# yoeripoels/neural-pde-surrogates

Hardware: AMD Instinct MI355X
Metric: rollout timesteps/sec on 256x256 two-phase grid (sample-timesteps/s); rel-L2 vs CPU reference (higher is better)
Workload: dtype f32 (1x1/2x2/3x3/5x5 convs: 3-pass split-fp16 MFMA); 1 GPU; UFNO twophase cfg rollout (simulate), 256x256, 3 fields, obstacle mask, tw=25; model=ufno, global_batch=16, per_gpu_batch=16, res=256, num_c=3, parallelism=dp1 (batch-sharded rollout, no collective)

## Files before the change

### neural-pde-surrogates_amd/csrc/conv2d_x3.hip

```cpp
#include "conv2d_common.hpp"

#include <cstdlib>
#include <type_traits>

namespace {

__host__ __device__ constexpr int x3_patch_px_max(int ntaps, int tile_px) {
    return ntaps == 1      ? tile_px
           : ntaps == 25   ? (tile_px == 512 ? 12 * 68 : 12 * 36)
           : tile_px == 128 ? (ntaps == 4 ? 5 * 33 : 6 * 34)
                            : (tile_px == 512 ? (ntaps == 4 ? 9 * 65 : 10 * 66) : (ntaps == 4 ? 9 * 33 : 10 * 34));
}

#define X3_MFMA __builtin_amdgcn_mfma_f32_32x32x16_f16
__device__ __forceinline__ int x3_slot_px(int idx) { return idx >> 2; }

template <int N, typename F>
__device__ __forceinline__ void static_for(F&& f) {
    if constexpr (N > 0) {
        static_for<N - 1>(f);
        f(std::integral_constant<int, N - 1>{});
    }
}

// ... 432 lines not shown
                        *reinterpret_cast<f32x4*>(T + P * (NCO + 4) + cw0 + cb * 32 + 8 * m + 4 * h) = v;
                    }
            }
            barrier();
            x3_store_phase<TILE_PX, NCO>(a, b, cob, oy0, ox0, g.T, ph, T, btab, tid, amax, reinterpret_cast<double*>(smem));
        } else if constexpr (!WIDE) {
            static_for<PBW>([&](auto pbc) {
                constexpr int pb = decltype(pbc)::value;
                const int P = px0 + pb * 32 + (lane & 31);
                const int ti = P / a.TW, tj = P - (P / a.TW) * a.TW;
                const int oy = oy0 + ti * g.T, ox = ox0 + tj * g.T;
                if (oy >= a.Hout || ox >= a.Wout) return;
                const int dy = oy * a.out_os + a.out_off_y + (ph >> 1), dx = ox * a.out_os + a.out_off_x + (ph & 1);
                if (dy < 0 || dy >= a.out_H || dx < 0 || dx >= a.out_W) return;
#pragma unroll
                for (int cb = 0; cb < CBW; ++cb) {
                    f32x16 v = acc[cb][pb];
#pragma unroll
                    for (int r = 0; r < 16; ++r) v[r] *= inv;
                    store_tile(a, b, cob * NCO + cw0 + cb * 32, h, v, dy, dx, amax);
                    __builtin_amdgcn_sched_barrier(0);
                }
            });
            barrier();
        }
        barrier();
    }
    nps::tag_publish(a.out_tag, amax, nps::wave_salt());
}



template <int PB, int D>
__global__ __launch_bounds__(512) void conv1x1_x3_kernel(const nps_conv2d_t a) {
    constexpr int CBW = 2;
    const int lane = threadIdx.x & 63, wv = threadIdx.x >> 6;
    const int co_lo = blockIdx.z * 512;
    const int cob = (co_lo >> 6) + wv;
    const int b = blockIdx.y;
    const int h = lane >> 5;
    const int npx = a.Hout * a.Wout;
    const int P0 = blockIdx.x * (PB * 32);
    const float xs = in_scale_of(a);
    const bool scaled = has_in_scale(a);
    int fy[PB], fx[PB];
    unsigned pin = 0;
#pragma unroll
    for (int pb = 0; pb < PB; ++pb) {
        const int P = P0 + pb * 32 + (lane & 31);
        const int oy = P / a.Wout, ox = P - (P / a.Wout) * a.Wout;
        const int ye = oy - a.pad_y, xe = ox - a.pad_x;
        const bool ok = P < npx && ye >= 0 && ye < a.Hin + 2 * a.circ && xe >= 0 && xe < a.Win + 2 * a.circ;
        fy[pb] = a.circ ? nps::wrap_mod(ye - a.circ, a.Hin) : ye;
        fx[pb] = a.circ ? nps::wrap_mod(xe - a.circ, a.Win) : xe;
        pin = ok ? (pin | (1u << pb)) : pin;
    }
    const float* sp[PB];
    int cur_src = -1;
    int cbase = 0;
    auto locate = [&](int sidx) {
        const nps_src_t S0 = a.src[0], S1 = a.src[1], S2 = a.src[2];
        const float* sptr = sidx == 0 ? S0.ptr : (sidx == 1 ? S1.ptr : S2.ptr);
        const int sC = sidx == 0 ? S0.C : (sidx == 1 ? S1.C : S2.C);
        const int sH = sidx == 0 ? S0.H : (sidx == 1 ? S1.H : S2.H);
        const int sW = sidx == 0 ? S0.W : (sidx == 1 ? S1.W : S2.W);
        const int soy = sidx == 0 ? S0.off_y : (sidx == 1 ? S1.off_y : S2.off_y);
        const int sox = sidx == 0 ? S0.off_x : (sidx == 1 ? S1.off_x : S2.off_x);
#pragma unroll
        for (int pb = 0; pb < PB; ++pb) {
            const int yy = fy[pb] - soy, xx = fx[pb] - sox;
            const bool ok = ((pin >> pb) & 1u) && yy >= 0 && yy < sH && xx >= 0 && xx < sW;
            sp[pb] = ok ? sptr + ((size_t)(b * sH + yy) * sW + xx) * sC : nullptr;
        }
    };
    const int nstages = (a.Cin + 2 * CK - 1) / (2 * CK);
    const int last = nstages - 1;
    f32x4 raw[D][PB][4];
    auto issue = [&](int st, bool live, f32x4 (&r)[PB][4]) {
        const int c0 = st * 2 * CK + h * CK;
        int sidx = 0, lo = 0, sb = 0;
#pragma unroll
        for (int si = 0; si < NPS_MAX_SRC; ++si) {
            if (si < a.nsrc) {
                const int hi = lo + a.src[si].C;
                if (c0 >= lo && c0 < hi) {
                    sidx = si;
                    sb = lo;
                }
                lo = hi;
            }
        }
        if (sidx != cur_src) {
            locate(sidx);
            cur_src = sidx;
            cbase = sb;
        }
#pragma unroll
        for (int q = 0; q < 4; ++q) {
            const bool chok = live && c0 + q * 4 < a.Cin;
#pragma unroll
            for (int pb = 0; pb < PB; ++pb) {
                const float* src = (chok && sp[pb] != nullptr) ? sp[pb] + (c0 - cbase + q * 4) : x3_zero16;
                r[pb][q] = *reinterpret_cast<const f32x4*>(src);
            }
        }
    };
    const int ncb = packed_ncb(a.Cout);
    const size_t gstride = (size_t)ncb * 2048;
    const int wcob = cob < ncb / CBW ? cob : ncb / CBW - 1;
    const char* wbase = reinterpret_cast<const char*>(a.wpack) + (size_t)wcob * CBW * 2048 + lane * 16;
    f16x8 Aw[2][2][CBW][2];
    auto loadA = [&](int st, f16x8 (&d)[2][CBW][2]) {
#pragma unroll
        for (int k = 0; k < 2; ++k) {
            const char* p = wbase + (size_t)(2 * st + k) * gstride;
#pragma unroll
            for (int cb = 0; cb < CBW; ++cb) {
                d[k][cb][0] = *reinterpret_cast<const f16x8*>(p + cb * 2048);
                d[k][cb][1] = *reinterpret_cast<const f16x8*>(p + cb * 2048 + 1024);
            }
        }
    };
    f32x16 acc[CBW][PB];
#pragma unroll
    for (int i = 0; i < CBW; ++i)
#pragma unroll
        for (int j = 0; j < PB; ++j)
#pragma unroll
            for (int r = 0; r < 16; ++r) acc[i][j][r] = 0.f;
    static_for<D - 1>([&](auto jc) {
        constexpr int j = decltype(jc)::value;
        issue(min(j, last), j <= last, raw[j]);
    });
    loadA(0, Aw[0]);
    const int npad = (nstages + D - 1) / D * D;
    for (int s0 = 0; s0 < npad; s0 += D) {
        static_for<D>([&](auto jc) {
            constexpr int j = decltype(jc)::value;
            constexpr int jn = (j + D - 1) % D;
            const int st = s0 + j;
            issue(min(st + D - 1, last), st + D - 1 <= last, raw[jn]);
            loadA(min(st + 1, last), Aw[(j + 1) & 1]);
            __builtin_amdgcn_sched_barrier(0);
            constexpr int r = j & 1;
#pragma unroll
            for (int k = 0; k < 2; ++k) {
                f16x8 Bh[PB], Bl[PB];
#pragma unroll
                for (int pb = 0; pb < PB; ++pb) {
                    f16x4 h0, l0, h1, l1;
                    f32x4 v0 = raw[j][pb][2 * k], v1 = raw[j][pb][2 * k + 1];
                    if (scaled) {
                        v0 *= xs;
                        v1 *= xs;
                    }
                    split4(v0, h0, l0);
                    split4(v1, h1, l1);
                    Bh[pb] = f16x8{h0[0], h0[1], h0[2], h0[3], h1[0], h1[1], h1[2], h1[3]};
                    Bl[pb] = f16x8{l0[0], l0[1], l0[2], l0[3], l1[0], l1[1], l1[2], l1[3]};
                }
#pragma unroll
                for (int cb = 0; cb < CBW; ++cb)
#pragma unroll
                    for (int pb = 0; pb < PB; ++pb)
                        acc[cb][pb] = X3_MFMA(Aw[r][k][cb][0], Bh[pb], acc[cb][pb], 0, 0, 0);
#pragma unroll
                for (int cb = 0; cb < CBW; ++cb)
#pragma unroll
                    for (int pb = 0; pb < PB; ++pb)
                        acc[cb][pb] = X3_MFMA(Aw[r][k][cb][0], Bl[pb], acc[cb][pb], 0, 0, 0);
#pragma unroll
                for (int cb = 0; cb < CBW; ++cb)
#pragma unroll
                    for (int pb = 0; pb < PB; ++pb)
                        acc[cb][pb] = X3_MFMA(Aw[r][k][cb][1], Bh[pb], acc[cb][pb], 0, 0, 0);
            }
        });
    }
    const float inv = 1.f / (pow2_scale_for(a.wpack[packed_body(a.Cout, a.Cin, 1)]) * xs);
    if (x3_lds_epilogue(a)) {
        extern __shared__ __attribute__((aligned(16))) float T[];
        const int pitch = (int)(blockDim.x) + 4;
#pragma unroll
        for (int pb = 0; pb < PB; ++pb) {
            const int P = pb * 32 + (lane & 31);
#pragma unroll
            for (int cb = 0; cb < CBW; ++cb)
#pragma unroll
                for (int m = 0; m < 4; ++m) {
                    const f32x4 v = {acc[cb][pb][4 * m] * inv, acc[cb][pb][4 * m + 1] * inv,
                                     acc[cb][pb][4 * m + 2] * inv, acc[cb][pb][4 * m + 3] * inv};
                    *reinterpret_cast<f32x4*>(T + P * pitch + wv * 64 + cb * 32 + 8 * m + 4 * h) = v;
                }
        }
        __syncthreads();
        const int nco = min(a.Cout - co_lo, (int)blockDim.x);
        const int C4 = nco >> 2;
        const bool fixq = ((int)blockDim.x % C4) == 0;
        const int pstep = fixq ? (int)blockDim.x / C4 : 0;
        int fp = fixq ? (int)threadIdx.x / C4 : 0;
        const int fcl = fixq ? ((int)threadIdx.x - fp * C4) * 4 : 0;
        int foy = (P0 + fp) / a.Wout, fox = (P0 + fp) - ((P0 + fp) / a.Wout) * a.Wout;
        float amax = 0.f;
        for (int i = threadIdx.x; i < PB * 32 * C4; i += blockDim.x) {
            int p, cl, oy, ox;
            if (fixq) {
                p = fp;
                cl = fcl;
                oy = foy;
                ox = fox;
                fp += pstep;
                fox += pstep;
                while (fox >= a.Wout) {
                    fox -= a.Wout;
                    ++foy;
                }
            } else {
                p = i / C4;
                cl = (i - (i / C4) * C4) * 4;
                oy = (P0 + p) / a.Wout;
                ox = (P0 + p) - ((P0 + p) / a.Wout) * a.Wout;
            }
            const int co0 = co_lo + cl;
            const int P = P0 + p;
            if (P >= npx) continue;
            const int dy = oy * a.out_os + a.out_off_y, dx = ox * a.out_os + a.out_off_x;
            if (dy < 0 || dy >= a.out_H || dx < 0 || dx >= a.out_W) continue;
            const f32x4 accv = *reinterpret_cast<const f32x4*>(T + p * pitch + cl);
            const size_t o = (((size_t)b * a.out_H + dy) * a.out_W + dx) * a.out_C + co0;
            const f32x4 z = {0.f, 0.f, 0.f, 0.f};
            const f32x4 bi = a.bias ? *reinterpret_cast<const f32x4*>(a.bias + co0) : z;
            const f32x4 a0 = a.addend0 ? *reinterpret_cast<const f32x4*>(a.addend0 + o) : z;
            const f32x4 a1 = a.addend1 ? *reinterpret_cast<const f32x4*>(a.addend1 + o) : z;
            const f32x4 ov = a.accumulate ? *reinterpret_cast<const f32x4*>(a.out + o) : z;
            f32x4 r;
#pragma unroll
            for (int e = 0; e < 4; ++e) {
                float v = accv[e] + bi[e];
                if (!a.add_after_act) v = v + a0[e] + a1[e];
                if (a.act == 1) v = nps::gelu_erf(v);
                if (a.add_after_act) v = v + a0[e] + a1[e];
                if (a.accumulate) v += ov[e];
                r[e] = v;
                amax = fmaxf(amax, fabsf(v));
            }
            *reinterpret_cast<f32x4*>(a.out + o) = r;
        }
        nps::tag_publish(a.out_tag, amax, nps::wave_salt());
        return;
    }
    float amax = 0.f;
    static_for<PB>([&](auto pbc) {
        constexpr int pb = decltype(pbc)::value;
        const int P = P0 + pb * 32 + (lane & 31);
        if (P >= npx) return;
        const int oy = P / a.Wout, ox = P - (P / a.Wout) * a.Wout;
        const int dy = oy * a.out_os + a.out_off_y, dx = ox * a.out_os + a.out_off_x;
        if (dy < 0 || dy >= a.out_H || dx < 0 || dx >= a.out_W) return;
#pragma unroll
        for (int cb = 0; cb < CBW; ++cb) {
            const int co = cob * 64 + cb * 32;
            if (co >= a.Cout) continue;
            f32x16 v = acc[cb][pb];
#pragma unroll
            for (int r = 0; r < 16; ++r) v[r] *= inv;
            store_tile(a, b, co, h, v, dy, dx, amax);
        }
    });
    nps::tag_publish(a.out_tag, amax, nps::wave_salt());
}

template <int NCB, int D, bool PRO = false>
__global__ __launch_bounds__(256) __attribute__((amdgpu_waves_per_eu(2))) void conv1x1_wl_kernel(const nps_conv2d_t a,
                                                                                                  int ng) {
    constexpr int WSTAGE = 2 * NCB * 2048;
    constexpr int WPT = WSTAGE / (256 * 16);
    static_assert(WSTAGE % (256 * 16) == 0, "weight stage split");
    extern __shared__ __attribute__((aligned(16))) char wl[];
    const int lane = threadIdx.x & 63, wv = threadIdx.x >> 6;
    const int b = blockIdx.y;
    const int h = lane >> 5;
    const int npx = a.Hout * a.Wout;
    int tile = (int)blockIdx.x, grp = 0;
    if (ng > 1) {
        const int r = (int)blockIdx.x >> 3;
        grp = r % ng;
        tile = (r / ng) * 8 + ((int)blockIdx.x & 7);
        if (tile * 128 >= npx) return;
    }
    const int cob = grp * NCB * 32;
    const int nact = min(NCB, (a.Cout - cob + 31) / 32);
    const int P = tile * 128 + wv * 32 + (lane & 31);
    const float xs = PRO ? gn_prologue_scale(a) : in_scale_of(a);
    const bool scaled = PRO || has_in_scale(a);
    int fy, fx;
    bool pin;
    {
        const int oy = P / a.Wout, ox = P - (P / a.Wout) * a.Wout;
        const int ye = oy - a.pad_y, xe = ox - a.pad_x;
        pin = P < npx && ye >= 0 && ye < a.Hin + 2 * a.circ && xe >= 0 && xe < a.Win + 2 * a.circ;
        fy = a.circ ? nps::wrap_mod(ye - a.circ, a.Hin) : ye;
        fx = a.circ ? nps::wrap_mod(xe - a.circ, a.Win) : xe;
    }
    const float* sp = nullptr;
    int cur_src = -1, cbase = 0;
    auto locate = [&](int sidx) {
        const nps_src_t S0 = a.src[0], S1 = a.src[1], S2 = a.src[2];
        const float* sptr = sidx == 0 ? S0.ptr : (sidx == 1 ? S1.ptr : S2.ptr);
        const int sC = sidx == 0 ? S0.C : (sidx == 1 ? S1.C : S2.C);
        const int sH = sidx == 0 ? S0.H : (sidx == 1 ? S1.H : S2.H);
        const int sW = sidx == 0 ? S0.W : (sidx == 1 ? S1.W : S2.W);
        const int yy = fy - (sidx == 0 ? S0.off_y : (sidx == 1 ? S1.off_y : S2.off_y));
        const int xx = fx - (sidx == 0 ? S0.off_x : (sidx == 1 ? S1.off_x : S2.off_x));
        const bool ok = pin && yy >= 0 && yy < sH && xx >= 0 && xx < sW;
        sp = ok ? sptr + ((size_t)(b * sH + yy) * sW + xx) * sC : nullptr;
    };
    const int nstages = (a.Cin + 2 * CK - 1) / (2 * CK);
    const int last = nstages - 1;
    f32x4 raw[D][4];
    auto issue = [&](int st, bool live, f32x4 (&r)[4]) {
        const int c0 = st * 2 * CK + h * CK;
        int sidx = 0, lo = 0, sb = 0;
#pragma unroll
        for (int si = 0; si < NPS_MAX_SRC; ++si) {
            if (si < a.nsrc) {
                const int hi = lo + a.src[si].C;
                if (c0 >= lo && c0 < hi) {
                    sidx = si;
                    sb = lo;
                }
                lo = hi;
            }
        }
        if (sidx != cur_src) {
            locate(sidx);
            cur_src = sidx;
            cbase = sb;
        }
#pragma unroll
        for (int q = 0; q < 4; ++q) {
            const bool chok = live && c0 + q * 4 < a.Cin;
            const float* src = (chok && sp != nullptr) ? sp + (c0 - cbase + q * 4) : x3_zero16;
            r[q] = *reinterpret_cast<const f32x4*>(src);
        }
    };
    const size_t gstride = (size_t)packed_ncb(a.Cout) * 2048;
    const char* wg = reinterpret_cast<const char*>(a.wpack) + (size_t)grp * NCB * 2048;
    f32x4 wr[WPT];
    auto wfetch = [&](int st) {
#pragma unroll
        for (int i = 0; i < WPT; ++i) {
            const int off = (i * 256 + (int)threadIdx.x) * 16;
            const int k = off / (NCB * 2048), rem = off - k * (NCB * 2048);
            wr[i] = *reinterpret_cast<const f32x4*>(wg + (size_t)(2 * st + k) * gstride + rem);
        }
    };
    auto wstore = [&](int buf) {
#pragma unroll
        for (int i = 0; i < WPT; ++i)
            *reinterpret_cast<f32x4*>(wl + buf * WSTAGE + (i * 256 + (int)threadIdx.x) * 16) = wr[i];
    };
    if ((int)threadIdx.x < NCB * 32)
        reinterpret_cast<float*>(wl + 2 * WSTAGE)[threadIdx.x] =
            (a.bias != nullptr && cob + (int)threadIdx.x < a.Cout) ? a.bias[cob + threadIdx.x] : 0.f;
    float* gtab = reinterpret_cast<float*>(wl + 2 * WSTAGE + NCB * 32 * 4);
    if constexpr (PRO) {
        const int ncp = ((a.Cin + 2 * CK - 1) / (2 * CK)) * 2 * CK;
        const bool gn = a.gn_stats != nullptr;
        const double icnt = gn ? 1.0 / ((double)(a.Cin / a.gn_groups) * a.Hin * a.Win) : 0.0;
        for (int c = threadIdx.x; c < ncp; c += 256) {
            float gs = 1.f, gb = 0.f;
            if (c >= a.Cin) {
                gs = 0.f;
            } else if (gn) {
                const double* st = a.gn_stats + ((size_t)b * a.gn_groups + c / (a.Cin / a.gn_groups)) * 2;
                const double mu = st[0] * icnt;
                double var = fma(st[1], icnt, -mu * mu);
                var = var < 0.0 ? 0.0 : var;
                const float rstd = __builtin_amdgcn_rsqf((float)(var + (double)a.gn_eps));
                gs = rstd * a.gn_gamma[c];
                gb = fmaf(-(float)mu, gs, a.gn_beta[c]);
            }
            gtab[c] = gs;
            gtab[ncp + c] = gb;
        }
    }
    f32x16 acc[NCB];
#pragma unroll
    for (int i = 0; i < NCB; ++i)
#pragma unroll
        for (int r = 0; r < 16; ++r) acc[i][r] = 0.f;
    static_for<D - 1>([&](auto jc) {
        constexpr int j = decltype(jc)::value;
        issue(min(j, last), j <= last, raw[j]);
    });
    wfetch(0);
    wstore(0);
    wfetch(min(1, last));
    __syncthreads();
    const int npad = (nstages + D - 1) / D * D;
    for (int s0 = 0; s0 < npad; s0 += D) {
        static_for<D>([&](auto jc) {
            constexpr int j = decltype(jc)::value;
            constexpr int jn = (j + D - 1) % D;
            const int st = s0 + j;
            wstore((st + 1) & 1);
            wfetch(min(st + 2, last));
            issue(min(st + D - 1, last), st + D - 1 <= last, raw[jn]);
            __builtin_amdgcn_sched_barrier(0);
            const char* wb = wl + (st & 1) * WSTAGE + lane * 16;
#pragma unroll
            for (int k = 0; k < 2; ++k) {
                f16x4 h0, l0, h1, l1;
                f32x4 v0 = raw[j][2 * k], v1 = raw[j][2 * k + 1];
                if constexpr (PRO) {
                    const int ncp = ((a.Cin + 2 * CK - 1) / (2 * CK)) * 2 * CK;
                    const bool live = pin && st <= last;
                    const int c = min(st, last) * 2 * CK + h * CK + 8 * k;
                    const f32x4 s0 = *reinterpret_cast<const f32x4*>(gtab + c);
                    const f32x4 s1 = *reinterpret_cast<const f32x4*>(gtab + c + 4);
                    const f32x4 b0 = *reinterpret_cast<const f32x4*>(gtab + ncp + c);
                    const f32x4 b1 = *reinterpret_cast<const f32x4*>(gtab + ncp + c + 4);
#pragma unroll
                    for (int e = 0; e < 4; ++e) {
                        float y0 = fmaf(v0[e], s0[e], b0[e]), y1 = fmaf(v1[e], s1[e], b1[e]);
                        if (a.pre_act == 1) {
                            y0 = nps::gelu_fast(y0);
                            y1 = nps::gelu_fast(y1);
                        }
                        v0[e] = live ? y0 : 0.f;
                        v1[e] = live ? y1 : 0.f;
                    }
                }
                if (scaled) {
                    v0 *= xs;
                    v1 *= xs;
                }
                split4(v0, h0, l0);
                split4(v1, h1, l1);
                const f16x8 Bh = f16x8{h0[0], h0[1], h0[2], h0[3], h1[0], h1[1], h1[2], h1[3]};
                const f16x8 Bl = f16x8{l0[0], l0[1], l0[2], l0[3], l1[0], l1[1], l1[2], l1[3]};
#pragma unroll
                for (int cb = 0; cb < NCB; ++cb) {
                    if (cb >= nact) break;
                    const f16x8 Ah = *reinterpret_cast<const f16x8*>(wb + (k * NCB + cb) * 2048);
                    const f16x8 Al = *reinterpret_cast<const f16x8*>(wb + (k * NCB + cb) * 2048 + 1024);
                    acc[cb] = X3_MFMA(Ah, Bh, acc[cb], 0, 0, 0);
                    acc[cb] = X3_MFMA(Ah, Bl, acc[cb], 0, 0, 0);
                    acc[cb] = X3_MFMA(Al, Bh, acc[cb], 0, 0, 0);
                }
            }
            __syncthreads();
        });
    }
    const float inv = 1.f / (pow2_scale_for(a.wpack[packed_body(a.Cout, a.Cin, 1)]) * xs);
    if constexpr (!PRO) {
        if (a.spec_z != nullptr) {
            const int m2 = a.spec_m2, K2 = 2 * m2;
            const int t0 = tile * 128, y0 = t0 / a.Wout, x0 = t0 - y0 * a.Wout;
            float* zs = reinterpret_cast<float*>(wl + 256);
            float* ts = zs + K2 * NCB * 32;
            const float fac = a.spec_scale / inv;
            const float2* zrow = reinterpret_cast<const float2*>(a.spec_z) + ((size_t)b * a.Hout + y0) * m2 * a.Cout;
            for (int i = threadIdx.x; i < m2 * NCB * 32; i += 256) {
                const int k = i / (NCB * 32), o = i - k * (NCB * 32);
                const bool self_conj = (k == 0) || (2 * k == a.Wout);
                const float cm = self_conj ? 1.f : 2.f;
                float2 z = make_float2(0.f, 0.f);
                if (o < a.Cout) z = zrow[(size_t)k * a.Cout + o];
                zs[(2 * k) * NCB * 32 + o] = z.x * cm * fac;
                zs[(2 * k + 1) * NCB * 32 + o] = self_conj ? 0.f : z.y * cm * fac;
            }
            for (int i = threadIdx.x; i < 128 * m2; i += 256) {
                const int p = i / m2, k = i - (i / m2) * m2;
                const int ph = (int)(((long)k * (x0 + p)) % a.Wout);
                float sn, cs;
                sincospif(2.0f * (float)ph / (float)a.Wout, &sn, &cs);
                ts[p * K2 + 2 * k] = cs;
                ts[p * K2 + 2 * k + 1] = -sn;
            }
            __syncthreads();
            const float* tl = ts + (wv * 32 + (lane & 31)) * K2 + h;
            for (int k = 0; k < m2; ++k) {
                const float bt = tl[2 * k];
#pragma unroll
                for (int cb = 0; cb < NCB; ++cb)
                    acc[cb] = __builtin_amdgcn_mfma_f32_32x32x2f32(zs[(2 * k + h) * NCB * 32 + cb * 32 + (lane & 31)], bt,
                                                                  acc[cb], 0, 0, 0);
            }
        }
    }
    const int oy = P / a.Wout, ox = P - (P / a.Wout) * a.Wout;
    const int dy = oy * a.out_os + a.out_off_y, dx = ox * a.out_os + a.out_off_x;
    float amax = 0.f;
    const bool pout = P < npx && dy >= 0 && dy < a.out_H && dx >= 0 && dx < a.out_W;
    if (x3_lds_epilogue(a) && a.addend1 == nullptr && !a.accumulate) {
        const float* btab = reinterpret_cast<const float*>(wl + 2 * WSTAGE);
        const size_t base = pout ? (((size_t)b * a.out_H + dy) * a.out_W + dx) * a.out_C : 0;
        double s1 = 0.0, s2 = 0.0;
        auto epi = [&](auto opc) {
            constexpr bool OP = decltype(opc)::value;
            f32x4 a0[4];
            auto load = [&](int cb) {
#pragma unroll
                for (int m = 0; m < 4; ++m) {
                    const int co0 = cob + cb * 32 + 8 * m + 4 * h;
                    const bool ok = pout && co0 < a.Cout;
                    a0[m] = *reinterpret_cast<const f32x4*>(ok ? a.addend0 + base + co0 : x3_zero16);
                }
            };
            if constexpr (OP) load(0);
            static_for<NCB>([&](auto cbc) {
                constexpr int cb = decltype(cbc)::value;
                float f1 = 0.f, f2 = 0.f;
#pragma unroll
                for (int m = 0; m < 4; ++m) {
                    const int co0 = cb * 32 + 8 * m + 4 * h;
                    const bool ok = pout && cob + co0 < a.Cout;
                    const f32x4 bi = *reinterpret_cast<const f32x4*>(btab + co0);
#pragma unroll
                    for (int e = 0; e < 4; ++e) {
                        float v = acc[cb][4 * m + e] * inv + bi[e];
                        if constexpr (OP) {
                            if (!a.add_after_act) v = v + a0[m][e];
                        }
                        if (a.act == 1) v = nps::gelu_erf(v);
                        if constexpr (OP) {
                            if (a.add_after_act) v = v + a0[m][e];
                        }
                        acc[cb][4 * m + e] = v;
                        amax = ok ? fmaxf(amax, fabsf(v)) : amax;
                        f1 += ok ? v : 0.f;
                        f2 += ok ? v * v : 0.f;
                    }
                }
                s1 += (double)f1;
                s2 += (double)f2;
                if constexpr (OP && cb + 1 < NCB) {
                    __builtin_amdgcn_sched_barrier(0);
                    load(cb + 1);
                }
                __builtin_amdgcn_sched_barrier(0);
#pragma unroll
                for (int m = 0; m < 4; ++m) {
                    const int co0 = cob + cb * 32 + 8 * m + 4 * h;
                    const bool ok = pout && co0 < a.Cout;
                    const f32x4 r = {acc[cb][4 * m], acc[cb][4 * m + 1], acc[cb][4 * m + 2], acc[cb][4 * m + 3]};
                    *reinterpret_cast<f32x4*>(ok ? a.out + base + co0 : x3_sink + 4 * lane) = r;
                }
                __builtin_amdgcn_sched_barrier(0);
            });
        };
        if (a.addend0 != nullptr)
            epi(std::true_type{});
        else
            epi(std::false_type{});
        publish_wg(a, b, amax, s1, s2, reinterpret_cast<double*>(wl));
        return;
    }
    if (pout) {
#pragma unroll
        for (int cb = 0; cb < NCB; ++cb) {
            if (cob + cb * 32 >= a.Cout) continue;
            f32x16 v = acc[cb];
#pragma unroll
            for (int r = 0; r < 16; ++r) v[r] *= inv;
            store_tile(a, b, cob + cb * 32, h, v, dy, dx, amax);
        }
    }
    nps::tag_publish(a.out_tag, amax, nps::wave_salt());
    if (a.out_stats != nullptr) {
        double s1 = 0.0, s2 = 0.0;
        if (pout) {
#pragma unroll
            for (int cb = 0; cb < NCB; ++cb) {
                if (cob + cb * 32 >= a.Cout) continue;
                float f1 = 0.f, f2 = 0.f;
#pragma unroll
                for (int m = 0; m < 4; ++m) {
                    const int co0 = cob + cb * 32 + 8 * m + 4 * h;
                    if (co0 >= a.Cout) continue;
                    const f32x4 z = {0.f, 0.f, 0.f, 0.f};
                    const f32x4 bi = a.bias ? *reinterpret_cast<const f32x4*>(a.bias + co0) : z;
#pragma unroll
                    for (int e = 0; e < 4; ++e) {
                        const float r = acc[cb][4 * m + e] * inv + bi[e];
                        f1 += r;
                        f2 += r * r;
                    }
                }
                s1 += (double)f1;
                s2 += (double)f2;
            }
        }
        stats_publish(a, b, s1, s2);
    }
}

template <int NT, int PB, bool PRO = false, bool WIDE = false>
void launch_x3_one(const nps_conv2d_t& a, unsigned nwg, int lds, hipStream_t s) {
    static bool attr_set = false;
    if (!attr_set) {
        (void)hipFuncSetAttribute((const void*)conv2d_x3_kernel<NT, PB, PRO, WIDE>,
                                  hipFuncAttributeMaxDynamicSharedMemorySize, 160 * 1024);
        attr_set = true;
    }
    conv2d_x3_kernel<NT, PB, PRO, WIDE><<<nwg, 512, lds, s>>>(a);
}



}


static const int g_x1_groups = [] {
    const char* e = getenv("NPS_X1_GROUPS");
    return (e != nullptr && e[0] == '0') ? 0 : 1;
}();

static long g_x3_grid_override = 0;

extern "C" int nps_x3_set_grid(long wgs) {
    g_x3_grid_override = wgs > 0 ? wgs : 0;
    return 0;
}

int nps_launch_conv2d_x3(const nps_conv2d_t& a, int lds, hipStream_t s) {
    const Geo g = make_geo(a);
    const bool wide = x3_wide_tile(a);
    const long nwg = (long)g.tiles_x * g.tiles_y * a.B * ((a.Cout + (wide ? 191 : 63)) / (wide ? 192 : 64)) *
                     (a.nphase > 1 ? a.nphase : 1);
    NPS_CHECK_ARG(a.nphase <= 1 || (a.nphase == 4 && a.KH * a.KW == 4 && a.out_os == 2 && a.phase_wstride > 0),
                  "conv2d_fwd (split-fp16): nphase = 4 is the k4/s2 transposed conv (2x2 phases, out_os 2)");
    NPS_CHECK_ARG(nwg < (1L << 31), "conv2d_fwd: grid too large");
    static int ncu = 0;
    if (ncu == 0) {
        int dev = 0, n = 0;
        if (hipGetDevice(&dev) != hipSuccess ||
            hipDeviceGetAttribute(&n, hipDeviceAttributeMultiprocessorCount, dev) != hipSuccess || n <= 0)
            n = 256;
        ncu = n;
    }
    static long per = -1;
    if (per < 0) {
        per = (ncu & ~7) > 0 ? (ncu & ~7) : ncu;
        const char* e = getenv("NPS_X3_GRID");
        if (e != nullptr && atol(e) > 0) per = atol(e);
    }
    const long pw = g_x3_grid_override > 0 ? g_x3_grid_override : per;
    const bool lds_epi = !a.out_nchw && (a.out_C & 3) == 0 && (a.Cout & 3) == 0;
    const unsigned grid = (unsigned)(pw < nwg ? pw : nwg);
    const bool p512 = a.TH * a.TW == 512;
    const bool pro = a.gn_stats != nullptr || a.pre_act != 0;
    if (a.KH * a.KW == 1) {
        NPS_CHECK_ARG(!pro || a.Cout <= 192, "conv2d_fwd (split-fp16): a 1x1 prologue needs the LDS-weight kernel "
                      "(Cout <= 192)");
        NPS_CHECK_ARG(a.spec_z == nullptr || a.Cout <= 192,
                      "conv2d_fwd (split-fp16 1x1): the fused c2r term needs the LDS-weight kernel");
        const int ncob = (a.Cout + 63) / 64;
        NPS_CHECK_ARG(a.out_stats == nullptr || (a.Cout <= 192 && !a.accumulate && a.addend1 == nullptr && lds_epi),
                      "conv2d_fwd (split-fp16 1x1): out_stats needs the LDS-weight kernel (Cout <= 192), an NHWC "
                      "4-aligned output and at most one addend, no accumulate");
        static int res_on = -1;
        if (res_on < 0) {
            const char* e = getenv("NPS_X1_RES");
            res_on = (e != nullptr && e[0] == '1') ? 1 : 0;
        }
        if (pro) {
            const long nb = ((long)a.Hout * a.Wout + 127) / 128;
            NPS_CHECK_ARG(nb < (1L << 31) && a.B < 65536, "conv2d_fwd: grid too large");
            const int ncp = ((a.Cin + 31) / 32) * 32;
            conv1x1_wl_kernel<6, 2, true><<<dim3((unsigned)nb, a.B), 256, 2 * 2 * 6 * 2048 + 6 * 32 * 4 + 2 * ncp * 4, s>>>(a, 1);
            NPS_CHECK_LAUNCH("conv2d_fwd (split-fp16 1x1, LDS weights, GroupNorm prologue)");
            return 0;
        }
        if (nps_launch_conv1x1_res(a, res_on, s)) return 0;
        if (a.Cout <= 192 || g_x1_groups) {
            const int ng = (a.Cout + 191) / 192;
            long nb = ((long)a.Hout * a.Wout + 127) / 128;
            if (ng > 1) nb = (nb + 7) / 8 * 8 * ng;
            NPS_CHECK_ARG(nb < (1L << 31) && a.B < 65536, "conv2d_fwd: grid too large");
            conv1x1_wl_kernel<6, 2><<<dim3((unsigned)nb, a.B), 256, 2 * 2 * 6 * 2048 + 6 * 32 * 4, s>>>(a, ng);
            NPS_CHECK_LAUNCH("conv2d_fwd (split-fp16 1x1, LDS weights)");
            return 0;
        }
        const int waves = ncob < 8 ? ncob : 8;
        const long nblk = ((long)a.Hout * a.Wout + 63) / 64;
        NPS_CHECK_ARG(nblk < (1L << 31) && a.B < 65536, "conv2d_fwd: grid too large");
        const dim3 grid1((unsigned)nblk, a.B, (ncob + 7) / 8);
        const int lds1 = lds_epi ? 64 * (64 * waves + 4) * 4 : 0;
        conv1x1_x3_kernel<2, 2><<<grid1, 64 * waves, lds1, s>>>(a);
        NPS_CHECK_LAUNCH("conv2d_fwd (split-fp16 1x1)");
        return 0;
    }
    if (wide) {
        if (a.KH * a.KW == 9)
            pro ? launch_x3_one<9, 2, true, true>(a, grid, lds, s) : launch_x3_one<9, 2, false, true>(a, grid, lds, s);
        else if (a.KH * a.KW == 4)
            launch_x3_one<4, 2, false, true>(a, grid, lds, s);
        else
            NPS_CHECK_ARG(false, "conv2d_fwd (split-fp16): wide tiles are 2x2 / 3x3 only");
        NPS_CHECK_LAUNCH("conv2d_fwd (split-fp16, wide)");
        return 0;
    }
    switch (a.KH * a.KW) {
        case 9:
            if (pro)
                p512 ? launch_x3_one<9, 4, true>(a, grid, lds, s) : launch_x3_one<9, 2, true>(a, grid, lds, s);
            else
                p512 ? launch_x3_one<9, 4>(a, grid, lds, s) : launch_x3_one<9, 2>(a, grid, lds, s);
            break;
        case 25:
            NPS_CHECK_ARG(!p512, "conv2d_fwd (split-fp16): 5x5 needs a 256-pixel tile");
            launch_x3_one<25, 2>(a, grid, lds, s);
            break;
        case 4: p512 ? launch_x3_one<4, 4>(a, grid, lds, s) : launch_x3_one<4, 2>(a, grid, lds, s); break;
        default: NPS_CHECK_ARG(false, "conv2d_fwd (split-fp16): unsupported tap count"); break;
    }
    NPS_CHECK_LAUNCH("conv2d_fwd (split-fp16)");
    return 0;
}

extern "C" long nps_conv2d_x3_weight_span(const nps_conv2d_t* ap) {
    NPS_CHECK_ARG(ap != nullptr && ap->precision == NPS_PREC_X3F16, "conv2d_x3_weight_span: split-fp16 args only");
    const nps_conv2d_t& a = *ap;
    const int nt = a.KH * a.KW;
    const long ncb = packed_ncb(a.Cout);
    const long gstride = ncb * 2048;
    long span = (long)(packed_body(a.Cout, a.Cin, nt) + 1) * 4;
    auto top = [&](long v) { span = v > span ? v : span; };
    if (nt == 1) {
        const long nst = (a.Cin + 2 * CK - 1) / (2 * CK);
        const char* e = getenv("NPS_X1_RES");
        const int all = (e != nullptr && e[0] == '1') ? 1 : 0;
        int rncb = 0, rng = 0, rnres = 0;
        const bool pro = a.gn_stats != nullptr || a.pre_act != 0;
        if (!pro && nps_conv1x1_res_plan(a, all, &rncb, &rng, &rnres)) {
            top((rnres - 1) * gstride + (long)rng * rncb * 2048);
        } else if (a.Cout <= 192 || g_x1_groups) {
            top((2 * nst - 1) * gstride + (long)((a.Cout + 191) / 192) * 6 * 2048);
        } else {
            top((2 * nst - 1) * gstride + ncb * 2048);
        }
    } else {
        const long nstages = (a.Cin + CK - 1) / CK;
        const long G = nstages * nt;
        const bool wide = x3_wide_tile(a);
        const long nco = wide ? 192 : 64;
        const long ncob = (a.Cout + nco - 1) / nco;
        top((G - 1) * gstride + ncob * (nco / 32) * 2048);
    }
    if (a.nphase > 1) span += (long)(a.nphase - 1) * a.phase_wstride * 4;
    return span;
}
```

Baseline: 4236 sample-timesteps/s.

## Use global_load_lds weight DMA and branchless source addressing in 1x1 LDS conv

The 1x1 LDS-weight conv kernel now loads weights straight into LDS with global_load_lds instead of staging them through registers. It replaces the barrier with a waitcnt that still allows in-flight activation loads. The per-stage source lookup becomes branchless, using precomputed base-pointer deltas and a coverage mask. A full-tile specialised main loop interleaves A-fragment loads, split-fp16 conversion and MFMAs, and the prefetch ring depth D rises from 2 to 3. The aim is to cut VGPR pressure and load latency on the critical path, at the cost of more raw-buffer registers and a hand-tuned waitcnt that must match the number of loads in flight.

```diff
diff --git a/neural-pde-surrogates_amd/csrc/conv2d_x3.hip b/neural-pde-surrogates_amd/csrc/conv2d_x3.hip
--- a/neural-pde-surrogates_amd/csrc/conv2d_x3.hip
+++ b/neural-pde-surrogates_amd/csrc/conv2d_x3.hip
@@ -758,63 +758,70 @@
         fy = a.circ ? nps::wrap_mod(ye - a.circ, a.Hin) : ye;
         fx = a.circ ? nps::wrap_mod(xe - a.circ, a.Win) : xe;
     }
-    const float* sp = nullptr;
-    int cur_src = -1, cbase = 0;
-    auto locate = [&](int sidx) {
+    static_assert(NPS_MAX_SRC == 3, "three frame sources");
+    typedef const __attribute__((address_space(1))) float* gfp;
+    unsigned long long pa0, pd1, pd2;
+    int okmask;
+    {
         const nps_src_t S0 = a.src[0], S1 = a.src[1], S2 = a.src[2];
-        const float* sptr = sidx == 0 ? S0.ptr : (sidx == 1 ? S1.ptr : S2.ptr);
-        const int sC = sidx == 0 ? S0.C : (sidx == 1 ? S1.C : S2.C);
-        const int sH = sidx == 0 ? S0.H : (sidx == 1 ? S1.H : S2.H);
-        const int sW = sidx == 0 ? S0.W : (sidx == 1 ? S1.W : S2.W);
-        const int yy = fy - (sidx == 0 ? S0.off_y : (sidx == 1 ? S1.off_y : S2.off_y));
-        const int xx = fx - (sidx == 0 ? S0.off_x : (sidx == 1 ? S1.off_x : S2.off_x));
-        const bool ok = pin && yy >= 0 && yy < sH && xx >= 0 && xx < sW;
-        sp = ok ? sptr + ((size_t)(b * sH + yy) * sW + xx) * sC : nullptr;
-    };
+        auto covers = [&](int sH, int sW, int oy, int ox, bool used) {
+            const int yy = fy - oy, xx = fx - ox;
+            return used && pin && yy >= 0 && yy < sH && xx >= 0 && xx < sW;
+        };
+        auto addr = [&](const float* sptr, int sC, int sH, int sW, int oy, int ox, int lo) {
+            return reinterpret_cast<unsigned long long>(sptr) +
+                   ((((long long)b * sH + (fy - oy)) * sW + (fx - ox)) * sC - lo) * 4;
+        };
+        const unsigned long long pa1 = addr(S1.ptr, S1.C, S1.H, S1.W, S1.off_y, S1.off_x, S0.C);
+        pa0 = addr(S0.ptr, S0.C, S0.H, S0.W, S0.off_y, S0.off_x, 0);
+        pd1 = pa1 - pa0;
+        pd2 = addr(S2.ptr, S2.C, S2.H, S2.W, S2.off_y, S2.off_x, S0.C + S1.C) - pa1;
+        okmask = (covers(S0.H, S0.W, S0.off_y, S0.off_x, true) ? 1 : 0) |
+                 (covers(S1.H, S1.W, S1.off_y, S1.off_x, a.nsrc > 1) ? 2 : 0) |
+                 (covers(S2.H, S2.W, S2.off_y, S2.off_x, a.nsrc > 2) ? 4 : 0);
+    }
+    const int clo1 = a.nsrc > 1 ? a.src[0].C : 0x7fffffff;
+    const int clo2 = a.nsrc > 2 ? a.src[0].C + a.src[1].C : 0x7fffffff;
+    gfp zero16;
+    {
+        const unsigned long long z = reinterpret_cast<unsigned long long>(x3_zero16);
+        const unsigned zl = __builtin_amdgcn_readfirstlane((unsigned)z);
+        const unsigned zh = __builtin_amdgcn_readfirstlane((unsigned)(z >> 32));
+        zero16 = (gfp)(((unsigned long long)zh << 32) | zl);
+    }
     const int nstages = (a.Cin + 2 * CK - 1) / (2 * CK);
     const int last = nstages - 1;
     f32x4 raw[D][4];
-    auto issue = [&](int st, bool live, f32x4 (&r)[4]) {
+    auto issue = [&](int st, bool live, f32x4 (&r)[4]) __attribute__((always_inline)) {
         const int c0 = st * 2 * CK + h * CK;
-        int sidx = 0, lo = 0, sb = 0;
-#pragma unroll
-        for (int si = 0; si < NPS_MAX_SRC; ++si) {
-            if (si < a.nsrc) {
-                const int hi = lo + a.src[si].C;
-                if (c0 >= lo && c0 < hi) {
-                    sidx = si;
-                    sb = lo;
-                }
-                lo = hi;
-            }
-        }
-        if (sidx != cur_src) {
-            locate(sidx);
-            cur_src = sidx;
-            cbase = sb;
-        }
+        const int sidx = (c0 >= clo1 ? 1 : 0) + (c0 >= clo2 ? 1 : 0);
+        const gfp sp = (gfp)(pa0 + (sidx >= 1 ? pd1 : 0ull) + (sidx >= 2 ? pd2 : 0ull));
+        const bool cov = ((okmask >> sidx) & 1) != 0;
 #pragma unroll
         for (int q = 0; q < 4; ++q) {
             const bool chok = live && c0 + q * 4 < a.Cin;
-            const float* src = (chok && sp != nullptr) ? sp + (c0 - cbase + q * 4) : x3_zero16;
-            r[q] = *reinterpret_cast<const f32x4*>(src);
+            const gfp src = (chok && cov) ? sp + (c0 + q * 4) : zero16;
+            r[q] = *(const __attribute__((address_space(1))) f32x4*)src;
         }
     };
     const size_t gstride = (size_t)packed_ncb(a.Cout) * 2048;
     const char* wg = reinterpret_cast<const char*>(a.wpack) + (size_t)grp * NCB * 2048;
-    f32x4 wr[WPT];
-    auto wfetch = [&](int st) {
+    auto wdma = [&](int st, int buf) {
 #pragma unroll
         for (int i = 0; i < WPT; ++i) {
-            const int off = (i * 256 + (int)threadIdx.x) * 16;
-            const int k = off / (NCB * 2048), rem = off - k * (NCB * 2048);
-            wr[i] = *reinterpret_cast<const f32x4*>(wg + (size_t)(2 * st + k) * gstride + rem);
+            static_assert((NCB * 2048) % 4096 == 0, "a 256-thread piece lies in one chunk");
+            const int k = (i * 4096) / (NCB * 2048);
+            const int rem = i * 4096 - k * (NCB * 2048) + (int)threadIdx.x * 16;
+            __builtin_amdgcn_global_load_lds((const void*)(wg + (size_t)(2 * st + k) * gstride + rem),
+                                             (__attribute__((address_space(3))) void*)(wl + buf * WSTAGE +
+                                                                                       (i * 256 + wv * 64) * 16),
+                                             16, 0, 0);
         }
     };
-    auto wstore = [&](int buf) {
-#pragma unroll
-        for (int i = 0; i < WPT; ++i)
-            *reinterpret_cast<f32x4*>(wl + buf * WSTAGE + (i * 256 + (int)threadIdx.x) * 16) = wr[i];
+    static_assert(D >= 3 && 4 * (D - 2) <= 15, "ring depth");
+    auto wsync = [&]() {
+        __builtin_amdgcn_s_waitcnt(0x0070 | (4 * (D - 2)));
+        __builtin_amdgcn_s_barrier();
     };
     if ((int)threadIdx.x < NCB * 32)
         reinterpret_cast<float*>(wl + 2 * WSTAGE)[threadIdx.x] =
@@ -846,69 +853,102 @@
     for (int i = 0; i < NCB; ++i)
 #pragma unroll
         for (int r = 0; r < 16; ++r) acc[i][r] = 0.f;
+    wdma(0, 0);
     static_for<D - 1>([&](auto jc) {
         constexpr int j = decltype(jc)::value;
         issue(min(j, last), j <= last, raw[j]);
     });
-    wfetch(0);
-    wstore(0);
-    wfetch(min(1, last));
-    __syncthreads();
+    __builtin_amdgcn_s_waitcnt(0x0070 | (4 * (D - 2)));
+    __builtin_amdgcn_s_barrier();
     const int npad = (nstages + D - 1) / D * D;
-    for (int s0 = 0; s0 < npad; s0 += D) {
-        static_for<D>([&](auto jc) {
-            constexpr int j = decltype(jc)::value;
-            constexpr int jn = (j + D - 1) % D;
-            const int st = s0 + j;
-            wstore((st + 1) & 1);
-            wfetch(min(st + 2, last));
-            issue(min(st + D - 1, last), st + D - 1 <= last, raw[jn]);
-            __builtin_amdgcn_sched_barrier(0);
-            const char* wb = wl + (st & 1) * WSTAGE + lane * 16;
-#pragma unroll
-            for (int k = 0; k < 2; ++k) {
-                f16x4 h0, l0, h1, l1;
-                f32x4 v0 = raw[j][2 * k], v1 = raw[j][2 * k + 1];
-                if constexpr (PRO) {
-                    const int ncp = ((a.Cin + 2 * CK - 1) / (2 * CK)) * 2 * CK;
-                    const bool live = pin && st <= last;
-                    const int c = min(st, last) * 2 * CK + h * CK + 8 * k;
-                    const f32x4 s0 = *reinterpret_cast<const f32x4*>(gtab + c);
-                    const f32x4 s1 = *reinterpret_cast<const f32x4*>(gtab + c + 4);
-                    const f32x4 b0 = *reinterpret_cast<const f32x4*>(gtab + ncp + c);
-                    const f32x4 b1 = *reinterpret_cast<const f32x4*>(gtab + ncp + c + 4);
-#pragma unroll
-                    for (int e = 0; e < 4; ++e) {
-                        float y0 = fmaf(v0[e], s0[e], b0[e]), y1 = fmaf(v1[e], s1[e], b1[e]);
-                        if (a.pre_act == 1) {
-                            y0 = nps::gelu_fast(y0);
-                            y1 = nps::gelu_fast(y1);
+    auto splitQ = [&](int st, int k, int q, const f32x4 (&rw)[4], f16x4& hi, f16x4& lo) __attribute__((always_inline)) {
+        f32x4 v = rw[2 * k + q];
+        if constexpr (PRO) {
+            const int ncp = ((a.Cin + 2 * CK - 1) / (2 * CK)) * 2 * CK;
+            const bool live = pin && st <= last;
+            const int c = min(st, last) * 2 * CK + h * CK + 8 * k + 4 * q;
+            const f32x4 sc = *reinterpret_cast<const f32x4*>(gtab + c);
+            const f32x4 sh = *reinterpret_cast<const f32x4*>(gtab + ncp + c);
+#pragma unroll
+            for (int e = 0; e < 4; ++e) {
+                float y = fmaf(v[e], sc[e], sh[e]);
+                if (a.pre_act == 1) y = nps::gelu_fast(y);
+                v[e] = live ? y : 0.f;
+            }
+        }
+        if (scaled) v *= xs;
+        split4(v, hi, lo);
+    };
+    auto cat8 = [](const f16x4 u, const f16x4 w) { return f16x8{u[0], u[1], u[2], u[3], w[0], w[1], w[2], w[3]}; };
+    auto mainloop = [&](auto fullc) {
+        constexpr bool FULL = decltype(fullc)::value;
+        for (int s0 = 0; s0 < npad; s0 += D) {
+            static_for<D>([&](auto jc) {
+                constexpr int j = decltype(jc)::value;
+                constexpr int jn = (j + D - 1) % D;
+                const int st = s0 + j;
+                wdma(min(st + 1, last), (st + 1) & 1);
+                __builtin_amdgcn_sched_barrier(0);
+                issue(min(st + D - 1, last), st + D - 1 <= last, raw[jn]);
+                __builtin_amdgcn_sched_barrier(0);
+                const char* wb = wl + (st & 1) * WSTAGE + lane * 16;
+                if (st > last) {
+                } else if constexpr (FULL) {
+                    f16x8 A[2][2], Bh[2], Bl[2];
+                    f16x4 qh[2], ql[2];
+                    auto loadA = [&](int i, f16x8 (&d)[2]) __attribute__((always_inline)) {
+                        d[0] = *reinterpret_cast<const f16x8*>(wb + i * 2048);
+                        d[1] = *reinterpret_cast<const f16x8*>(wb + i * 2048 + 1024);
+                    };
+                    loadA(0, A[0]);
+                    splitQ(st, 0, 0, raw[j], qh[0], ql[0]);
+                    splitQ(st, 0, 1, raw[j], qh[1], ql[1]);
+                    Bh[0] = cat8(qh[0], qh[1]);
+                    Bl[0] = cat8(ql[0], ql[1]);
+                    __builtin_amdgcn_sched_barrier(0);
+                    static_for<2 * NCB>([&](auto ic) {
+                        constexpr int i = decltype(ic)::value;
+                        constexpr int k = i / NCB, cb = i - k * NCB;
+                        acc[cb] = X3_MFMA(A[i & 1][0], Bh[k], acc[cb], 0, 0, 0);
+                        __builtin_amdgcn_sched_barrier(0);
+                        if constexpr (i + 1 < 2 * NCB) loadA(i + 1, A[(i + 1) & 1]);
+                        __builtin_amdgcn_sched_barrier(0);
+                        if constexpr (i == 0) splitQ(st, 1, 0, raw[j], qh[0], ql[0]);
+                        if constexpr (i == 2) {
+                            splitQ(st, 1, 1, raw[j], qh[1], ql[1]);
+                            Bh[1] = cat8(qh[0], qh[1]);
+                            Bl[1] = cat8(ql[0], ql[1]);
                         }
-                        v0[e] = live ? y0 : 0.f;
-                        v1[e] = live ? y1 : 0.f;
+                        acc[cb] = X3_MFMA(A[i & 1][0], Bl[k], acc[cb], 0, 0, 0);
+                        acc[cb] = X3_MFMA(A[i & 1][1], Bh[k], acc[cb], 0, 0, 0);
+                        __builtin_amdgcn_sched_barrier(0);
+                    });
+                } else {
+#pragma unroll
+                    for (int k = 0; k < 2; ++k) {
+                        f16x4 h0, l0, h1, l1;
+                        splitQ(st, k, 0, raw[j], h0, l0);
+                        splitQ(st, k, 1, raw[j], h1, l1);
+                        const f16x8 Bh = cat8(h0, h1), Bl = cat8(l0, l1);
+#pragma unroll
+                        for (int cb = 0; cb < NCB; ++cb) {
+                            if (cb >= nact) break;
+                            const f16x8 Ah = *reinterpret_cast<const f16x8*>(wb + (k * NCB + cb) * 2048);
+                            const f16x8 Al = *reinterpret_cast<const f16x8*>(wb + (k * NCB + cb) * 2048 + 1024);
+                            acc[cb] = X3_MFMA(Ah, Bh, acc[cb], 0, 0, 0);
+                            acc[cb] = X3_MFMA(Ah, Bl, acc[cb], 0, 0, 0);
+                            acc[cb] = X3_MFMA(Al, Bh, acc[cb], 0, 0, 0);
+                        }
                     }
                 }
-                if (scaled) {
-                    v0 *= xs;
-                    v1 *= xs;
-                }
-                split4(v0, h0, l0);
-                split4(v1, h1, l1);
-                const f16x8 Bh = f16x8{h0[0], h0[1], h0[2], h0[3], h1[0], h1[1], h1[2], h1[3]};
-                const f16x8 Bl = f16x8{l0[0], l0[1], l0[2], l0[3], l1[0], l1[1], l1[2], l1[3]};
-#pragma unroll
-                for (int cb = 0; cb < NCB; ++cb) {
-                    if (cb >= nact) break;
-                    const f16x8 Ah = *reinterpret_cast<const f16x8*>(wb + (k * NCB + cb) * 2048);
-                    const f16x8 Al = *reinterpret_cast<const f16x8*>(wb + (k * NCB + cb) * 2048 + 1024);
-                    acc[cb] = X3_MFMA(Ah, Bh, acc[cb], 0, 0, 0);
-                    acc[cb] = X3_MFMA(Ah, Bl, acc[cb], 0, 0, 0);
-                    acc[cb] = X3_MFMA(Al, Bh, acc[cb], 0, 0, 0);
-                }
-            }
-            __syncthreads();
-        });
-    }
+                wsync();
+            });
+        }
+    };
+    if (nact == NCB)
+        mainloop(std::true_type{});
+    else
+        mainloop(std::false_type{});
     const float inv = 1.f / (pow2_scale_for(a.wpack[packed_body(a.Cout, a.Cin, 1)]) * xs);
     if constexpr (!PRO) {
         if (a.spec_z != nullptr) {
@@ -1126,7 +1166,7 @@
             const long nb = ((long)a.Hout * a.Wout + 127) / 128;
             NPS_CHECK_ARG(nb < (1L << 31) && a.B < 65536, "conv2d_fwd: grid too large");
             const int ncp = ((a.Cin + 31) / 32) * 32;
-            conv1x1_wl_kernel<6, 2, true><<<dim3((unsigned)nb, a.B), 256, 2 * 2 * 6 * 2048 + 6 * 32 * 4 + 2 * ncp * 4, s>>>(a, 1);
+            conv1x1_wl_kernel<6, 3, true><<<dim3((unsigned)nb, a.B), 256, 2 * 2 * 6 * 2048 + 6 * 32 * 4 + 2 * ncp * 4, s>>>(a, 1);
             NPS_CHECK_LAUNCH("conv2d_fwd (split-fp16 1x1, LDS weights, GroupNorm prologue)");
             return 0;
         }
@@ -1136,7 +1176,7 @@
             long nb = ((long)a.Hout * a.Wout + 127) / 128;
             if (ng > 1) nb = (nb + 7) / 8 * 8 * ng;
             NPS_CHECK_ARG(nb < (1L << 31) && a.B < 65536, "conv2d_fwd: grid too large");
-            conv1x1_wl_kernel<6, 2><<<dim3((unsigned)nb, a.B), 256, 2 * 2 * 6 * 2048 + 6 * 32 * 4, s>>>(a, ng);
+            conv1x1_wl_kernel<6, 3><<<dim3((unsigned)nb, a.B), 256, 2 * 2 * 6 * 2048 + 6 * 32 * 4, s>>>(a, ng);
             NPS_CHECK_LAUNCH("conv2d_fwd (split-fp16 1x1, LDS weights)");
             return 0;
         }
```

New measurement: 4323 sample-timesteps/s (median of 6 runs). 1.02x the previous value.
